# JackWoo0831/Yolov7-tracker

Measured on AMD Instinct MI355X. Metric: end-to-end fps (detect+track) YOLOv7-w6@1280 ByteTrack, higher is better.
Workload: dtype f16

## Files before the change

yolov7-tracker_amd/csrc/y7t_conv_p8.hip:

```cpp
#include "y7t_common.h"
#include "y7t_conv_common.h"
#include <stdlib.h>

namespace {

#if defined(Y7T_CONVSIM)
#define P8_VMCNT(n) cs_vmcnt(n)
#define P8_WAVE_SYNC() cs_wave_barrier(threadIdx.x >> 6)
#define P8_KEEP(a, b) ((void)0)
#else
#define P8_VMCNT(n) asm volatile("s_waitcnt vmcnt(" #n ")" ::: "memory")
#define P8_WAVE_SYNC() ((void)0)
#define P8_KEEP(a, b) asm volatile("" :: "v"(a), "v"(b))
#endif

struct P8 {
    static constexpr int BM = 256, BN = 256, BK = 64, NT = 512;
    static constexpr int ROWB = 128;
    static constexpr int HALF = 128 * ROWB;
    static constexpr int BUF = 4 * HALF;
    static constexpr int RING = 2 * BUF;
    static constexpr int BIAS = RING;
    static constexpr int LDS = RING + BN * 4;
    static constexpr unsigned OOB = 0xFF000000u;
};

template <int ACT, bool DUAL, int ABL = 0>
__global__ void __launch_bounds__(512, 2) k_conv1x1_p8(const Y7TConvArgs p) {
#if defined(__HIP_DEVICE_COMPILE__)
    using C = P8;
    extern __shared__ __attribute__((aligned(16))) char smem[];
    const int tid = threadIdx.x, lane = tid & 63, wave = tid >> 6;
    const int grp = wave >> 2, wq = wave & 3, l31 = lane & 31, hi32 = lane >> 5;

    int bid = blockIdx.x;
    if (p.xcd_swizzle) {
        const int nwg = gridDim.x, q = nwg >> 3, r = nwg & 7, xcd = bid & 7, idx = bid >> 3;
        bid = (xcd < r ? xcd * (q + 1) : r * (q + 1) + (xcd - r) * q) + idx;
    }
    const int n_tiles_n = p.Cout_pad / C::BN;
    const int tile_n = bid % n_tiles_n, tile_m = bid / n_tiles_n;
    const int m0 = tile_m * C::BM, n0 = tile_n * C::BN;
    const int nk = p.Cin / C::BK;

    const __amdgpu_buffer_rsrc_t xr = __builtin_amdgcn_make_buffer_rsrc((void*)p.in, 0, p.in_bytes, 0x00020000);
    const __amdgpu_buffer_rsrc_t wr = __builtin_amdgcn_make_buffer_rsrc((void*)p.w, 0, p.w_bytes, 0x00020000);
    const __amdgpu_buffer_rsrc_t br = __builtin_amdgcn_make_buffer_rsrc((void*)p.bias, 0, (unsigned)p.Cout_pad * 4u, 0x00020000);
    const __amdgpu_buffer_rsrc_t xr2 = __builtin_amdgcn_make_buffer_rsrc((void*)(DUAL ? p.in2 : p.in), 0, DUAL ? p.in2_bytes : p.in_bytes, 0x00020000);

    const int srow = wave * 8 + (lane >> 3);
    const int gch = (lane & 7) ^ ((srow >> 1) & 7);
    int xoff[2][2], xoff2[DUAL ? 2 : 1][2];
#pragma unroll
    for (int h = 0; h < 2; ++h)
#pragma unroll
        for (int rd = 0; rd < 2; ++rd) {
            const int m = m0 + rd * 128 + h * 64 + srow;
            xoff[h][rd] = (int)C::OOB;
            if (DUAL) xoff2[h][rd] = (int)C::OOB;
            if (m < p.M) {
                xoff[h][rd] = (m * p.ldin + p.cin_off + gch * 8) * 2;
                if (DUAL) {
                    const int HW = p.H * p.W, b = m / HW, rem = m - b * HW, y = rem / p.W, x = rem - y * p.W;
                    xoff2[h][rd] = (((b * (p.H >> 1) + (y >> 1)) * (p.W >> 1) + (x >> 1)) * p.ldin2 + p.cin2_off + gch * 8) * 2;
                }
            }
        }
    const int wvo = tile_n * nk * (2 * C::HALF) + wave * 1024 + lane * 16;

    bool in_loop = false;
    auto stage_p1 = [&](int h, int b, int T, int rd) __attribute__((always_inline)) {
        if ((ABL & 1) && in_loop) return;
        char* dst = smem + b * C::BUF + h * C::HALF + wave * 1024 + rd * 8192;
        const bool live = T < nk;
        const int ci = T * C::BK;
        const bool up = DUAL && live && ci >= p.up_c0 && ci < p.up_c0 + p.up_C;
        if (up) __builtin_amdgcn_raw_ptr_buffer_load_lds(xr2, (LDS_AS void*)dst, 16, xoff2[DUAL ? h : 0][rd], (ci - p.up_c0) * 2, 0, 0);
        else __builtin_amdgcn_raw_ptr_buffer_load_lds(xr, (LDS_AS void*)dst, 16, live ? xoff[h][rd] : (int)C::OOB, live ? ci * 2 : 0, 0, 0);
    };
    auto stage_c1 = [&](int h, int b, int T, int rd) __attribute__((always_inline)) {
        if ((ABL & 1) && in_loop) return;
        char* dst = smem + b * C::BUF + (2 + h) * C::HALF + wave * 1024 + rd * 8192;
        const bool live = T < nk;
        __builtin_amdgcn_raw_ptr_buffer_load_lds(wr, (LDS_AS void*)dst, 16, live ? wvo + h * C::HALF + rd * 8192 : (int)C::OOB, live ? T * (2 * C::HALF) : 0, 0, 0);
    };
    auto stage_p = [&](int h, int b, int T) __attribute__((always_inline)) { stage_p1(h, b, T, 0); stage_p1(h, b, T, 1); };
    auto stage_c = [&](int h, int b, int T) __attribute__((always_inline)) { stage_c1(h, b, T, 0); stage_c1(h, b, T, 1); };

    const int swl = (l31 >> 1) & 7;
    const int prow = (grp * 64 + l31) * C::ROWB, crow = (wq * 32 + l31) * C::ROWB;
    half8 pf[2][4], c0[4], c1[4];
    auto read_p = [&](int hP, int b) __attribute__((always_inline)) {
        if (ABL & 4) return;
#pragma unroll
        for (int j = 0; j < 2; ++j)
#pragma unroll
            for (int ks = 0; ks < 4; ++ks) pf[j][ks] = *(const half8*)(smem + b * C::BUF + hP * C::HALF + prow + j * 32 * C::ROWB + (((ks * 2 + hi32) ^ swl) << 4));
    };
    auto read_c = [&](half8 (&cf)[4], int hC, int b) __attribute__((always_inline)) {
        if (ABL & 4) return;
#pragma unroll
        for (int ks = 0; ks < 4; ++ks) cf[ks] = *(const half8*)(smem + b * C::BUF + (2 + hC) * C::HALF + crow + (((ks * 2 + hi32) ^ swl) << 4));
    };
    floatx16 acc[2][2][2];
    auto mma = [&](int hP, const half8 (&cf)[4], int hC) __attribute__((always_inline)) {
        if (!(ABL & 8)) __builtin_amdgcn_s_setprio(1);
#pragma unroll
        for (int ks = 0; ks < 4; ++ks)
#pragma unroll
            for (int j = 0; j < 2; ++j) {
                if (ABL & 2) P8_KEEP(cf[ks], pf[j][ks]);
                else acc[hP][j][hC] = __builtin_amdgcn_mfma_f32_32x32x16_f16(cf[ks], pf[j][ks], acc[hP][j][hC], 0, 0, 0);
            }
        if (!(ABL & 8)) __builtin_amdgcn_s_setprio(0);
    };

    __builtin_amdgcn_raw_ptr_buffer_load_lds(br, (LDS_AS void*)(smem + C::BIAS + wq * 256), 4, (n0 + wq * 64 + lane) * 4, 0, 0, 0);
    stage_p(0, 0, 0); stage_c(0, 0, 0); stage_c(1, 0, 0); stage_p(1, 0, 0); stage_p(0, 1, 1); stage_c(0, 1, 1);
    P8_VMCNT(8);
    __builtin_amdgcn_s_barrier();
#pragma unroll
    for (int hC = 0; hC < 2; ++hC)
#pragma unroll
        for (int g = 0; g < 4; ++g) {
            typedef __attribute__((ext_vector_type(4))) float float4v;
            const float4v bv = *(const float4v*)(smem + C::BIAS + (wq * 64 + hC * 32 + 8 * g + 4 * hi32) * 4);
#pragma unroll
            for (int hP = 0; hP < 2; ++hP)
#pragma unroll
                for (int j = 0; j < 2; ++j)
#pragma unroll
                    for (int e = 0; e < 4; ++e) acc[hP][j][hC][g * 4 + e] = bv[e];
        }
    if (grp == 1) __builtin_amdgcn_s_barrier();
    in_loop = true;
    if (ABL & 4) {
#pragma unroll
        for (int ks = 0; ks < 4; ++ks) { c0[ks] = c1[ks] = pf[0][ks] = pf[1][ks] = half8{1, 1, 1, 1, 1, 1, 1, 1}; }
    }

    auto ktile = [&](int T, auto bc) __attribute__((always_inline)) {
        constexpr int b = decltype(bc)::value;
        read_p(0, b); read_c(c0, 0, b);
        stage_c(1, b ^ 1, T + 1);
        P8_VMCNT(8);
        __builtin_amdgcn_s_barrier();
        mma(0, c0, 0);
        __builtin_amdgcn_s_barrier();
        read_c(c1, 1, b);
        stage_p(1, b ^ 1, T + 1);
        P8_VMCNT(8);
        __builtin_amdgcn_s_barrier();
        mma(0, c1, 1);
        __builtin_amdgcn_s_barrier();
        read_p(1, b);
        stage_p(0, b, T + 2);
        P8_VMCNT(8);
        __builtin_amdgcn_s_barrier();
        mma(1, c1, 1);
        __builtin_amdgcn_s_barrier();
        stage_c(0, b, T + 2);
        P8_VMCNT(8);
        __builtin_amdgcn_s_barrier();
        mma(1, c0, 0);
        __builtin_amdgcn_s_barrier();
    };
    for (int T = 0; T < nk; T += 2) {
        ktile(T, std::integral_constant<int, 0>{});
        if (T + 1 < nk) ktile(T + 1, std::integral_constant<int, 1>{});
    }
    if (grp == 0) __builtin_amdgcn_s_barrier();
    P8_VMCNT(0);
    __builtin_amdgcn_s_barrier();

    char* scr = smem + wave * 16384;
    typedef __attribute__((ext_vector_type(4))) unsigned uint4v;
#pragma unroll
    for (int hP = 0; hP < 2; ++hP)
#pragma unroll
        for (int j = 0; j < 2; ++j) {
            const int pl = hP * 64 + j * 32 + l31;
#pragma unroll
            for (int hC = 0; hC < 2; ++hC)
#pragma unroll
                for (int gp = 0; gp < 2; ++gp) {
                    unsigned w[2][2];
#pragma unroll
                    for (int gg = 0; gg < 2; ++gg) {
                        const int g = gp * 2 + gg;
                        float v[4];
#pragma unroll
                        for (int e = 0; e < 4; ++e) v[e] = act_t<ACT>(acc[hP][j][hC][g * 4 + e]);
                        typedef __attribute__((ext_vector_type(2))) _Float16 half2v;
                        half2v h0 = {(half_t)v[0], (half_t)v[1]}, h1 = {(half_t)v[2], (half_t)v[3]};
                        w[gg][0] = __builtin_bit_cast(unsigned, h0);
                        w[gg][1] = __builtin_bit_cast(unsigned, h1);
                    }
                    auto r0 = __builtin_amdgcn_permlane32_swap(w[0][0], w[1][0], false, false);
                    auto r1 = __builtin_amdgcn_permlane32_swap(w[0][1], w[1][1], false, false);
                    uint4v pk = {r0[0], r1[0], r0[1], r1[1]};
                    const int ch = hC * 4 + gp * 2 + hi32;
                    *(uint4v*)(scr + pl * 128 + ((ch ^ (pl & 7)) << 4)) = pk;
                }
        }
    P8_WAVE_SYNC();
    half_t* outp = (half_t*)p.out;
#pragma unroll 1
    for (int k0 = 0; k0 < 16; k0 += 8) {
        uint4v v[8];
#pragma unroll
        for (int k = 0; k < 8; ++k) {
            const int px = (k0 + k) * 8 + (lane >> 3), ch = lane & 7;
            v[k] = *(const uint4v*)(scr + px * 128 + ((ch ^ (px & 7)) << 4));
        }
        __builtin_amdgcn_sched_barrier(0);
#pragma unroll
        for (int k = 0; k < 8; ++k) {
            const int px = (k0 + k) * 8 + (lane >> 3), ch = lane & 7;
            const int m = m0 + grp * 128 + px, n = n0 + wq * 64 + ch * 8;
            if (m < p.M && n < p.Cout && !(ABL & 16)) *(uint4v*)(outp + (size_t)m * p.ldout + p.cout_off + n) = v[k];
        }
    }
#endif
}


template <int ACT, bool DUAL, bool DYN>
__global__ void __launch_bounds__(512, 2) k_conv1x1_p8p(const Y7TConvArgs p) {
#if defined(__HIP_DEVICE_COMPILE__)
    using C = P8;
    extern __shared__ __attribute__((aligned(16))) char smem[];
    const int tid = threadIdx.x, lane = tid & 63, wave = tid >> 6;
    const int grp = wave >> 2, wq = wave & 3, l31 = lane & 31, hi32 = lane >> 5;
    int bid = blockIdx.x;
    if (p.xcd_swizzle) {
        const int nwg = gridDim.x, q = nwg >> 3, r = nwg & 7, xcd = bid & 7, idx = bid >> 3;
        bid = (xcd < r ? xcd * (q + 1) : r * (q + 1) + (xcd - r) * q) + idx;
    }
    const int n_tiles_n = p.Cout_pad / C::BN, Gn = (int)gridDim.x / n_tiles_n;
    const int tile_n = bid % n_tiles_n, m_tiles = (p.M + C::BM - 1) / C::BM;
    int tile_m = bid / n_tiles_n;
    if (tile_m >= m_tiles) return;
    const int n0 = tile_n * C::BN, nk = p.Cin / C::BK;

    const __amdgpu_buffer_rsrc_t xr = __builtin_amdgcn_make_buffer_rsrc((void*)p.in, 0, p.in_bytes, 0x00020000);
    const __amdgpu_buffer_rsrc_t wr = __builtin_amdgcn_make_buffer_rsrc((void*)p.w, 0, p.w_bytes, 0x00020000);
    const __amdgpu_buffer_rsrc_t br = __builtin_amdgcn_make_buffer_rsrc((void*)p.bias, 0, (unsigned)p.Cout_pad * 4u, 0x00020000);
    const __amdgpu_buffer_rsrc_t xr2 = __builtin_amdgcn_make_buffer_rsrc((void*)(DUAL ? p.in2 : p.in), 0, DUAL ? p.in2_bytes : p.in_bytes, 0x00020000);

    const int srow = wave * 8 + (lane >> 3);
    const int gch = (lane & 7) ^ ((srow >> 1) & 7);
    struct Off { int x[2][2]; int x2[DUAL ? 2 : 1][2]; };
    auto offsets = [&](int m0, Off& o) __attribute__((always_inline)) {
#pragma unroll
        for (int h = 0; h < 2; ++h)
#pragma unroll
            for (int rd = 0; rd < 2; ++rd) {
                const int m = m0 + rd * 128 + h * 64 + srow;
                o.x[h][rd] = (int)C::OOB;
                if (DUAL) o.x2[h][rd] = (int)C::OOB;
                if (m < p.M) {
                    o.x[h][rd] = (m * p.ldin + p.cin_off + gch * 8) * 2;
                    if (DUAL) {
                        const int HW = p.H * p.W, b = m / HW, rem = m - b * HW, y = rem / p.W, x = rem - y * p.W;
                        o.x2[h][rd] = (((b * (p.H >> 1) + (y >> 1)) * (p.W >> 1) + (x >> 1)) * p.ldin2 + p.cin2_off + gch * 8) * 2;
                    }
                }
            }
    };
    Off cur, nxt;
    bool has_next = false;
    volatile int* const tkt = (volatile int*)(smem + C::LDS);
    int* const ctr = DYN ? p.tile_ctr + tile_n : nullptr;
    if (DYN && tid == 0) tkt[0] = atomicAdd(ctr, 1);
    const int wvo = tile_n * nk * (2 * C::HALF) + wave * 1024 + lane * 16;

    auto stage_p1 = [&](int h, int b, int T, int rd) __attribute__((always_inline)) {
        char* dst = smem + b * C::BUF + h * C::HALF + wave * 1024 + rd * 8192;
        const bool own = T < nk, live = own || has_next;
        const int ci = (own ? T : T - nk) * C::BK;
        const bool up = DUAL && live && ci >= p.up_c0 && ci < p.up_c0 + p.up_C;
        const int xo = own ? cur.x[h][rd] : nxt.x[h][rd];
        if (up) __builtin_amdgcn_raw_ptr_buffer_load_lds(xr2, (LDS_AS void*)dst, 16, own ? cur.x2[DUAL ? h : 0][rd] : nxt.x2[DUAL ? h : 0][rd], (ci - p.up_c0) * 2, 0, 0);
        else __builtin_amdgcn_raw_ptr_buffer_load_lds(xr, (LDS_AS void*)dst, 16, live ? xo : (int)C::OOB, live ? ci * 2 : 0, 0, 0);
    };
    auto stage_c1 = [&](int h, int b, int T, int rd) __attribute__((always_inline)) {
        char* dst = smem + b * C::BUF + (2 + h) * C::HALF + wave * 1024 + rd * 8192;
        const bool own = T < nk, live = own || has_next;
        const int Tw = own ? T : T - nk;
        __builtin_amdgcn_raw_ptr_buffer_load_lds(wr, (LDS_AS void*)dst, 16, live ? wvo + h * C::HALF + rd * 8192 : (int)C::OOB, live ? Tw * (2 * C::HALF) : 0, 0, 0);
    };
    auto stage_p = [&](int h, int b, int T) __attribute__((always_inline)) { stage_p1(h, b, T, 0); stage_p1(h, b, T, 1); };
    auto stage_c = [&](int h, int b, int T) __attribute__((always_inline)) { stage_c1(h, b, T, 0); stage_c1(h, b, T, 1); };

    const int swl = (l31 >> 1) & 7;
    const int prow = (grp * 64 + l31) * C::ROWB, crow = (wq * 32 + l31) * C::ROWB;
    half8 pf[2][4], c0[4], c1[4];
    auto read_p = [&](int hP, int b) __attribute__((always_inline)) {
#pragma unroll
        for (int j = 0; j < 2; ++j)
#pragma unroll
            for (int ks = 0; ks < 4; ++ks) pf[j][ks] = *(const half8*)(smem + b * C::BUF + hP * C::HALF + prow + j * 32 * C::ROWB + (((ks * 2 + hi32) ^ swl) << 4));
    };
    auto read_c = [&](half8 (&cf)[4], int hC, int b) __attribute__((always_inline)) {
#pragma unroll
        for (int ks = 0; ks < 4; ++ks) cf[ks] = *(const half8*)(smem + b * C::BUF + (2 + hC) * C::HALF + crow + (((ks * 2 + hi32) ^ swl) << 4));
    };
    floatx16 acc[2][2][2];
    auto mma = [&](int hP, const half8 (&cf)[4], int hC) __attribute__((always_inline)) {
        __builtin_amdgcn_s_setprio(1);
#pragma unroll
        for (int ks = 0; ks < 4; ++ks)
#pragma unroll
            for (int j = 0; j < 2; ++j) acc[hP][j][hC] = __builtin_amdgcn_mfma_f32_32x32x16_f16(cf[ks], pf[j][ks], acc[hP][j][hC], 0, 0, 0);
        __builtin_amdgcn_s_setprio(0);
    };
    auto ktile = [&](int T, auto bc) __attribute__((always_inline)) {
        constexpr int b = decltype(bc)::value;
        read_p(0, b); read_c(c0, 0, b);
        stage_c(1, b ^ 1, T + 1);
        P8_VMCNT(8);
        __builtin_amdgcn_s_barrier();
        mma(0, c0, 0);
        __builtin_amdgcn_s_barrier();
        read_c(c1, 1, b);
        stage_p(1, b ^ 1, T + 1);
        P8_VMCNT(8);
        __builtin_amdgcn_s_barrier();
        mma(0, c1, 1);
        __builtin_amdgcn_s_barrier();
        read_p(1, b);
        stage_p(0, b, T + 2);
        P8_VMCNT(8);
        __builtin_amdgcn_s_barrier();
        mma(1, c1, 1);
        __builtin_amdgcn_s_barrier();
        stage_c(0, b, T + 2);
        P8_VMCNT(8);
        __builtin_amdgcn_s_barrier();
        mma(1, c0, 0);
        __builtin_amdgcn_s_barrier();
    };

    offsets(tile_m * C::BM, cur);
    __builtin_amdgcn_raw_ptr_buffer_load_lds(br, (LDS_AS void*)(smem + C::BIAS + wq * 256), 4, (n0 + wq * 64 + lane) * 4, 0, 0, 0);
    stage_p(0, 0, 0); stage_c(0, 0, 0); stage_c(1, 0, 0); stage_p(1, 0, 0); stage_p(0, 1, 1); stage_c(0, 1, 1);
    P8_VMCNT(8);
    __builtin_amdgcn_s_barrier();
    typedef __attribute__((ext_vector_type(4))) unsigned uint4v;
    half_t* outp = (half_t*)p.out;
    char* const scr = smem + C::BUF + (wave < 4 ? 1 : 3) * C::HALF + (wave & 3) * 4096;
    for (int it = 0;; ++it) {
        const int m0 = tile_m * C::BM, tile_next = DYN ? Gn + __builtin_amdgcn_readfirstlane(tkt[it & 1]) : tile_m + Gn;
        has_next = tile_next < m_tiles;
        int fetched = 0;
        if (DYN && tid == 0 && has_next) {
#if defined(Y7T_CONVSIM)
            fetched = atomicAdd(ctr, 1);
#else
            asm volatile("global_atomic_add %0, %1, %2, off sc0" : "=v"(fetched) : "v"(ctr), "v"(1) : "memory");
#endif
        }
        if (has_next) offsets(tile_next * C::BM, nxt);
#pragma unroll
        for (int hC = 0; hC < 2; ++hC)
#pragma unroll
            for (int g = 0; g < 4; ++g) {
                typedef __attribute__((ext_vector_type(4))) float float4v;
                const float4v bv = *(const float4v*)(smem + C::BIAS + (wq * 64 + hC * 32 + 8 * g + 4 * hi32) * 4);
#pragma unroll
                for (int hP = 0; hP < 2; ++hP)
#pragma unroll
                    for (int j = 0; j < 2; ++j)
#pragma unroll
                        for (int e = 0; e < 4; ++e) acc[hP][j][hC][g * 4 + e] = bv[e];
            }
        if (grp == 1) __builtin_amdgcn_s_barrier();
        for (int T = 0; T < nk; T += 2) {
            ktile(T, std::integral_constant<int, 0>{});
            ktile(T + 1, std::integral_constant<int, 1>{});
        }
        if (grp == 0) __builtin_amdgcn_s_barrier();
        if (DYN && tid == 0 && has_next) tkt[(it + 1) & 1] = fetched;
#pragma unroll
        for (int hP = 0; hP < 2; ++hP)
#pragma unroll
            for (int j = 0; j < 2; ++j) {
#pragma unroll
                for (int hC = 0; hC < 2; ++hC)
#pragma unroll
                    for (int gp = 0; gp < 2; ++gp) {
                        unsigned w[2][2];
#pragma unroll
                        for (int gg = 0; gg < 2; ++gg) {
                            const int g = gp * 2 + gg;
                            float v[4];
#pragma unroll
                            for (int e = 0; e < 4; ++e) v[e] = act_t<ACT>(acc[hP][j][hC][g * 4 + e]);
                            typedef __attribute__((ext_vector_type(2))) _Float16 half2v;
                            half2v h0 = {(half_t)v[0], (half_t)v[1]}, h1 = {(half_t)v[2], (half_t)v[3]};
                            w[gg][0] = __builtin_bit_cast(unsigned, h0);
                            w[gg][1] = __builtin_bit_cast(unsigned, h1);
                        }
                        auto r0 = __builtin_amdgcn_permlane32_swap(w[0][0], w[1][0], false, false);
                        auto r1 = __builtin_amdgcn_permlane32_swap(w[0][1], w[1][1], false, false);
                        uint4v pk = {r0[0], r1[0], r0[1], r1[1]};
                        const int ch = hC * 4 + gp * 2 + hi32;
                        *(uint4v*)(scr + l31 * 128 + ((ch ^ (l31 & 7)) << 4)) = pk;
                    }
                P8_WAVE_SYNC();
                uint4v v4[4];
#pragma unroll
                for (int k = 0; k < 4; ++k) {
                    const int px = k * 8 + (lane >> 3), ch = lane & 7;
                    v4[k] = *(const uint4v*)(scr + px * 128 + ((ch ^ (px & 7)) << 4));
                }
                __builtin_amdgcn_sched_barrier(0);
#pragma unroll
                for (int k = 0; k < 4; ++k) {
                    const int px = k * 8 + (lane >> 3), ch = lane & 7;
                    const int m = m0 + grp * 128 + hP * 64 + j * 32 + px, n = n0 + wq * 64 + ch * 8;
                    if (m < p.M && n < p.Cout) *(uint4v*)(outp + (size_t)m * p.ldout + p.cout_off + n) = v4[k];
                }
                P8_WAVE_SYNC();
            }
        if (!has_next) break;
        __builtin_amdgcn_s_barrier();
        cur = nxt;
        tile_m = tile_next;
    }
    P8_VMCNT(0);
    if (DYN && tid == 0) {
        if (atomicAdd(p.tile_ctr + Y7T_TILE_CTR_DONE, 1) == (int)gridDim.x - 1) {
            for (int i = 0; i <= Y7T_TILE_CTR_DONE; ++i) p.tile_ctr[i] = 0;
        }
    }
#endif
}

}

int y7t_conv_p8_launch(const Y7TConvArgs& a, hipStream_t s) {
    using C = P8;
    bool ok = a.KH == 1 && a.KW == 1 && a.stride == 1 && a.pad == 0 && a.Cin % C::BK == 0 && a.K_pad == a.Cin && a.Cout_pad % C::BN == 0 && !a.out_f32 && !a.epi &&
              !(a.Cout & 7) && !(a.ldout & 7) && !(a.cout_off & 7) && !(a.ldin & 7) && !(a.cin_off & 7) && a.in_bytes <= C::OOB - (1u << 24) && a.Ho == a.H && a.Wo == a.W;
    if (a.up_C > 0) ok = ok && a.up_c0 % C::BK == 0 && a.up_C % C::BK == 0 && a.up_c0 + a.up_C <= a.Cin && !(a.H & 1) && !(a.W & 1) && !(a.ldin2 & 7) && !(a.cin2_off & 7) &&
                         a.in2_bytes <= C::OOB - (1u << 24);
    if (!ok) {
        y7t_set_error("conv: weights are in the 256 x 64 panel order (korder 7) but the layer is not a 1x1 / stride 1 convolution with Cin %% 64 == 0, Cout_pad %% 256 == 0 "
                      "and an aligned fp16 output (Cin=%d Cout=%d Cout_pad=%d ldout=%d cout_off=%d up=[%d,%d))", a.Cin, a.Cout, a.Cout_pad, a.ldout, a.cout_off, a.up_c0,
                      a.up_c0 + a.up_C);
        return Y7T_E_ARG;
    }
    static Y7TOncePerDevice attr;
    if (int e_ = y7t_once_per_device(attr, [&]() -> int {
#define P8_ATTR(ACT, DUAL) Y7T_HIP_CHECK(hipFuncSetAttribute((const void*)k_conv1x1_p8<ACT, DUAL>, hipFuncAttributeMaxDynamicSharedMemorySize, C::LDS));
        P8_ATTR(Y7T_ACT_NONE, false) P8_ATTR(Y7T_ACT_SILU, false) P8_ATTR(Y7T_ACT_LEAKY, false) P8_ATTR(Y7T_ACT_NONE, true) P8_ATTR(Y7T_ACT_SILU, true) P8_ATTR(Y7T_ACT_LEAKY, true)
#undef P8_ATTR
        return 0;
    })) return e_;
    const int grid = ((a.M + C::BM - 1) / C::BM) * (a.Cout_pad / C::BN);
    const bool dual = a.up_C > 0;
    static const int persist = y7t_exp_switch("Y7T_CONV_P8_PERSIST", 1);
    const int n_tiles_n = a.Cout_pad / C::BN, ncu = y7t_num_cus(), gp_ = (ncu / n_tiles_n) * n_tiles_n;
    if (persist && !a.ablate && ((a.Cin / C::BK) & 1) == 0 && gp_ > 0 && grid >= 2 * gp_) {
        static Y7TOncePerDevice attrp;
        if (int e_ = y7t_once_per_device(attrp, [&]() -> int {
#define P8P_ATTR(ACT, DUAL) Y7T_HIP_CHECK(hipFuncSetAttribute((const void*)k_conv1x1_p8p<ACT, DUAL, false>, hipFuncAttributeMaxDynamicSharedMemorySize, C::LDS + 16)); \
                            Y7T_HIP_CHECK(hipFuncSetAttribute((const void*)k_conv1x1_p8p<ACT, DUAL, true>, hipFuncAttributeMaxDynamicSharedMemorySize, C::LDS + 16));
            P8P_ATTR(Y7T_ACT_NONE, false) P8P_ATTR(Y7T_ACT_SILU, false) P8P_ATTR(Y7T_ACT_LEAKY, false) P8P_ATTR(Y7T_ACT_NONE, true) P8P_ATTR(Y7T_ACT_SILU, true) P8P_ATTR(Y7T_ACT_LEAKY, true)
#undef P8P_ATTR
            return 0;
        })) return e_;
        static const int dyn_env = y7t_switch("Y7T_CONV_WS_DYN", 1);
        const bool dyn = a.tile_ctr && dyn_env && n_tiles_n <= Y7T_TILE_CTR_DONE;
#define P8P_GO(ACT) \
        do { if (dual && dyn) hipLaunchKernelGGL((k_conv1x1_p8p<ACT, true, true>), dim3(gp_), dim3(C::NT), C::LDS + 16, s, a); \
             else if (dual) hipLaunchKernelGGL((k_conv1x1_p8p<ACT, true, false>), dim3(gp_), dim3(C::NT), C::LDS + 16, s, a); \
             else if (dyn) hipLaunchKernelGGL((k_conv1x1_p8p<ACT, false, true>), dim3(gp_), dim3(C::NT), C::LDS + 16, s, a); \
             else hipLaunchKernelGGL((k_conv1x1_p8p<ACT, false, false>), dim3(gp_), dim3(C::NT), C::LDS + 16, s, a); } while (0)
        if (a.act == Y7T_ACT_SILU) P8P_GO(Y7T_ACT_SILU);
        else if (a.act == Y7T_ACT_LEAKY) P8P_GO(Y7T_ACT_LEAKY);
        else P8P_GO(Y7T_ACT_NONE);
#undef P8P_GO
        Y7T_LAUNCH_CHECK();
        y7t_note_kernel("p8<256,256,64> 1x1%s", dual ? " upsample-on-read" : "");
        return 0;
    }
#if Y7T_ABLATE
    if (a.ablate && a.act == Y7T_ACT_SILU && !dual) {
#define P8_ABL(N) case N: Y7T_HIP_CHECK(hipFuncSetAttribute((const void*)k_conv1x1_p8<Y7T_ACT_SILU, false, N>, hipFuncAttributeMaxDynamicSharedMemorySize, C::LDS)); \
                          hipLaunchKernelGGL((k_conv1x1_p8<Y7T_ACT_SILU, false, N>), dim3(grid), dim3(C::NT), C::LDS, s, a); break;
        switch (a.ablate) { P8_ABL(1) P8_ABL(2) P8_ABL(4) P8_ABL(8) P8_ABL(16) P8_ABL(6) P8_ABL(7) default: y7t_set_error("conv: unknown p8 ablation %d", a.ablate); return Y7T_E_ARG; }
#undef P8_ABL
        Y7T_LAUNCH_CHECK();
        y7t_note_kernel("p8<256,256,64> 1x1 ablated");
        return 0;
    }
#endif
#define P8_GO(ACT) \
    do { if (dual) hipLaunchKernelGGL((k_conv1x1_p8<ACT, true>), dim3(grid), dim3(C::NT), C::LDS, s, a); \
         else hipLaunchKernelGGL((k_conv1x1_p8<ACT, false>), dim3(grid), dim3(C::NT), C::LDS, s, a); } while (0)
    if (a.act == Y7T_ACT_SILU) P8_GO(Y7T_ACT_SILU);
    else if (a.act == Y7T_ACT_LEAKY) P8_GO(Y7T_ACT_LEAKY);
    else P8_GO(Y7T_ACT_NONE);
#undef P8_GO
    Y7T_LAUNCH_CHECK();
    y7t_note_kernel("p8<256,256,64> 1x1%s", dual ? " upsample-on-read" : "");
    return 0;
}
```

Before: 2456.

## Interleave SiLU epilogue math into the last k-tile's MFMA gaps

For SiLU-activated 1x1 conv kernels, the last k-tile now applies the activation to already-final accumulator quadrants between MFMA issues. A compile-time micro-program table spreads the exp, rcp and multiply steps across the gaps of the 8 MFMAs per phase, and the epilogue skips those elements. This is meant to hide part of the epilogue's transcendental work behind matrix-core latency. The persistent kernel also moves bias re-initialization into the store loop and makes the wave index scalar via readfirstlane. The cost is added code complexity, scheduling barriers that constrain the compiler, and more register pressure from temporaries.

```diff
diff --git a/yolov7-tracker_amd/csrc/y7t_conv_p8.hip b/yolov7-tracker_amd/csrc/y7t_conv_p8.hip
--- a/yolov7-tracker_amd/csrc/y7t_conv_p8.hip
+++ b/yolov7-tracker_amd/csrc/y7t_conv_p8.hip
@@ -8,10 +8,12 @@
 #define P8_VMCNT(n) cs_vmcnt(n)
 #define P8_WAVE_SYNC() cs_wave_barrier(threadIdx.x >> 6)
 #define P8_KEEP(a, b) ((void)0)
+#define P8_PIN(x) ((void)0)
 #else
 #define P8_VMCNT(n) asm volatile("s_waitcnt vmcnt(" #n ")" ::: "memory")
 #define P8_WAVE_SYNC() ((void)0)
 #define P8_KEEP(a, b) asm volatile("" :: "v"(a), "v"(b))
+#define P8_PIN(x) asm volatile("" : "+v"(x))
 #endif
 
 struct P8 {
@@ -25,12 +27,68 @@
     static constexpr unsigned OOB = 0xFF000000u;
 };
 
+struct P8EA {
+    static constexpr int L = 4, G = 6;
+    static constexpr int PER_PHASE = L + G, N = 3 * PER_PHASE;
+    static_assert(L >= 0 && G >= 0 && PER_PHASE <= 32, "a phase may only touch quadrants that are final");
+    enum { EX, M1, RC, AD, M2 };
+    static constexpr int NOPS = 5 * (G + 3);
+    struct Tbl { signed char gap[NOPS], val[NOPS]; int last; };
+    static constexpr Tbl make() {
+        Tbl t{};
+        constexpr int dv[5] = {0, 1, -1, 0, -2}, cost[5] = {8, 4, 8, 4, 4};
+        int gap = 0, used = 0;
+        for (int o = 0; o < NOPS; ++o) {
+            const int k = o % 5, v = o / 5 - 1 + dv[k];
+            t.val[o] = (signed char)v;
+            t.gap[o] = -1;
+            if (v < 0 || v >= G) continue;
+            if (used + cost[k] > 24) { ++gap; used = 0; }
+            used += cost[k];
+            t.gap[o] = (signed char)gap;
+        }
+        t.last = gap;
+        return t;
+    }
+    static constexpr int index(int hP, int j, int hC, int e) { return ((hP == 0 ? hC : 3 - hC) * 2 + j) * 16 + e; }
+};
+static_assert(P8EA::make().last <= 7, "the micro-program of a phase fits the gaps of its 8 MFMAs");
+typedef floatx16 P8Acc[2][2][2];
+__device__ __forceinline__ float p8_ea_get(const P8Acc& acc, int n) { const int q = n >> 5; return acc[q >> 1][(n >> 4) & 1][q == 1 || q == 2][n & 15]; }
+__device__ __forceinline__ void p8_ea_set(P8Acc& acc, int n, float y) { const int q = n >> 5; acc[q >> 1][(n >> 4) & 1][q == 1 || q == 2][n & 15] = y; }
+__device__ __forceinline__ void p8_ea_load(P8Acc& acc, int ph) {
+#pragma unroll
+    for (int i = 0; i < P8EA::L; ++i) {
+        const int n = (ph - 1) * P8EA::PER_PHASE + i;
+        float y = act_t<Y7T_ACT_SILU>(p8_ea_get(acc, n));
+        P8_PIN(y);
+        p8_ea_set(acc, n, y);
+    }
+}
+__device__ __forceinline__ void p8_ea_gap(P8Acc& acc, float (&t)[P8EA::G > 0 ? P8EA::G : 1], int ph, int g) {
+    constexpr P8EA::Tbl tbl = P8EA::make();
+#pragma unroll
+    for (int o = 0; o < P8EA::NOPS; ++o) {
+        if (tbl.gap[o] != g) continue;
+        const int v = tbl.val[o], n = (ph - 1) * P8EA::PER_PHASE + P8EA::L + v;
+        switch (o % 5) {
+            case P8EA::M1: t[v] = -1.44269504088896f * p8_ea_get(acc, n); break;
+            case P8EA::EX: t[v] = __builtin_amdgcn_exp2f(t[v]); break;
+            case P8EA::AD: t[v] = 1.0f + t[v]; break;
+            case P8EA::RC: t[v] = __builtin_amdgcn_rcpf(t[v]); break;
+            default: t[v] = p8_ea_get(acc, n) * t[v]; break;
+        }
+        P8_PIN(t[v]);
+        if (o % 5 == P8EA::M2) p8_ea_set(acc, n, t[v]);
+    }
+}
+
 template <int ACT, bool DUAL, int ABL = 0>
 __global__ void __launch_bounds__(512, 2) k_conv1x1_p8(const Y7TConvArgs p) {
 #if defined(__HIP_DEVICE_COMPILE__)
     using C = P8;
     extern __shared__ __attribute__((aligned(16))) char smem[];
-    const int tid = threadIdx.x, lane = tid & 63, wave = tid >> 6;
+    const int tid = threadIdx.x, lane = tid & 63, wave = __builtin_amdgcn_readfirstlane(tid >> 6);
     const int grp = wave >> 2, wq = wave & 3, l31 = lane & 31, hi32 = lane >> 5;
 
     int bid = blockIdx.x;
@@ -102,7 +160,7 @@
 #pragma unroll
         for (int ks = 0; ks < 4; ++ks) cf[ks] = *(const half8*)(smem + b * C::BUF + (2 + hC) * C::HALF + crow + (((ks * 2 + hi32) ^ swl) << 4));
     };
-    floatx16 acc[2][2][2];
+    P8Acc acc;
     auto mma = [&](int hP, const half8 (&cf)[4], int hC) __attribute__((always_inline)) {
         if (!(ABL & 8)) __builtin_amdgcn_s_setprio(1);
 #pragma unroll
@@ -114,6 +172,25 @@
             }
         if (!(ABL & 8)) __builtin_amdgcn_s_setprio(0);
     };
+    constexpr bool EA = ACT == Y7T_ACT_SILU && ABL == 0 && P8EA::N > 0;
+    float eat[P8EA::G > 0 ? P8EA::G : 1];
+    auto mma_ea = [&](int hP, const half8 (&cf)[4], int hC, int ph) __attribute__((always_inline)) {
+        __builtin_amdgcn_s_setprio(1);
+#pragma unroll
+        for (int ks = 0; ks < 4; ++ks)
+#pragma unroll
+            for (int j = 0; j < 2; ++j) {
+                acc[hP][j][hC] = __builtin_amdgcn_mfma_f32_32x32x16_f16(cf[ks], pf[j][ks], acc[hP][j][hC], 0, 0, 0);
+                p8_ea_gap(acc, eat, ph, ks * 2 + j);
+                __builtin_amdgcn_sched_barrier(0);
+            }
+        __builtin_amdgcn_s_setprio(0);
+    };
+    auto ea_load = [&](int ph) __attribute__((always_inline)) {
+        __builtin_amdgcn_sched_barrier(0);
+        p8_ea_load(acc, ph);
+        __builtin_amdgcn_sched_barrier(0);
+    };
 
     __builtin_amdgcn_raw_ptr_buffer_load_lds(br, (LDS_AS void*)(smem + C::BIAS + wq * 256), 4, (n0 + wq * 64 + lane) * 4, 0, 0, 0);
     stage_p(0, 0, 0); stage_c(0, 0, 0); stage_c(1, 0, 0); stage_p(1, 0, 0); stage_p(0, 1, 1); stage_c(0, 1, 1);
@@ -139,8 +216,9 @@
         for (int ks = 0; ks < 4; ++ks) { c0[ks] = c1[ks] = pf[0][ks] = pf[1][ks] = half8{1, 1, 1, 1, 1, 1, 1, 1}; }
     }
 
-    auto ktile = [&](int T, auto bc) __attribute__((always_inline)) {
-        constexpr int b = decltype(bc)::value;
+    auto ktile = [&](int T, auto bc, auto lc) __attribute__((always_inline)) {
+        const int b = bc;
+        constexpr bool LAST = EA && decltype(lc)::value;
         read_p(0, b); read_c(c0, 0, b);
         stage_c(1, b ^ 1, T + 1);
         P8_VMCNT(8);
@@ -149,25 +227,32 @@
         __builtin_amdgcn_s_barrier();
         read_c(c1, 1, b);
         stage_p(1, b ^ 1, T + 1);
-        P8_VMCNT(8);
-        __builtin_amdgcn_s_barrier();
-        mma(0, c1, 1);
+        if (LAST) ea_load(1);
+        P8_VMCNT(8);
+        __builtin_amdgcn_s_barrier();
+        if (LAST) mma_ea(0, c1, 1, 1); else mma(0, c1, 1);
         __builtin_amdgcn_s_barrier();
         read_p(1, b);
         stage_p(0, b, T + 2);
-        P8_VMCNT(8);
-        __builtin_amdgcn_s_barrier();
-        mma(1, c1, 1);
+        if (LAST) ea_load(2);
+        P8_VMCNT(8);
+        __builtin_amdgcn_s_barrier();
+        if (LAST) mma_ea(1, c1, 1, 2); else mma(1, c1, 1);
         __builtin_amdgcn_s_barrier();
         stage_c(0, b, T + 2);
-        P8_VMCNT(8);
-        __builtin_amdgcn_s_barrier();
-        mma(1, c0, 0);
-        __builtin_amdgcn_s_barrier();
-    };
-    for (int T = 0; T < nk; T += 2) {
-        ktile(T, std::integral_constant<int, 0>{});
-        if (T + 1 < nk) ktile(T + 1, std::integral_constant<int, 1>{});
+        if (LAST) ea_load(3);
+        P8_VMCNT(8);
+        __builtin_amdgcn_s_barrier();
+        if (LAST) mma_ea(1, c0, 0, 3); else mma(1, c0, 0);
+        __builtin_amdgcn_s_barrier();
+    };
+    {
+        constexpr std::integral_constant<int, 0> B0{};
+        constexpr std::integral_constant<int, 1> B1{};
+        int T = 0;
+        for (; T + 2 < nk; T += 2) { ktile(T, B0, std::false_type{}); ktile(T + 1, B1, std::false_type{}); }
+        if (T + 1 < nk) { ktile(T, B0, std::false_type{}); ++T; }
+        ktile(T, T & 1, std::true_type{});
     }
     if (grp == 0) __builtin_amdgcn_s_barrier();
     P8_VMCNT(0);
@@ -190,7 +275,7 @@
                         const int g = gp * 2 + gg;
                         float v[4];
 #pragma unroll
-                        for (int e = 0; e < 4; ++e) v[e] = act_t<ACT>(acc[hP][j][hC][g * 4 + e]);
+                        for (int e = 0; e < 4; ++e) v[e] = EA && P8EA::index(hP, j, hC, g * 4 + e) < P8EA::N ? acc[hP][j][hC][g * 4 + e] : act_t<ACT>(acc[hP][j][hC][g * 4 + e]);
                         typedef __attribute__((ext_vector_type(2))) _Float16 half2v;
                         half2v h0 = {(half_t)v[0], (half_t)v[1]}, h1 = {(half_t)v[2], (half_t)v[3]};
                         w[gg][0] = __builtin_bit_cast(unsigned, h0);
@@ -230,7 +315,7 @@
 #if defined(__HIP_DEVICE_COMPILE__)
     using C = P8;
     extern __shared__ __attribute__((aligned(16))) char smem[];
-    const int tid = threadIdx.x, lane = tid & 63, wave = tid >> 6;
+    const int tid = threadIdx.x, lane = tid & 63, wave = __builtin_amdgcn_readfirstlane(tid >> 6);
     const int grp = wave >> 2, wq = wave & 3, l31 = lane & 31, hi32 = lane >> 5;
     int bid = blockIdx.x;
     if (p.xcd_swizzle) {
@@ -306,7 +391,7 @@
 #pragma unroll
         for (int ks = 0; ks < 4; ++ks) cf[ks] = *(const half8*)(smem + b * C::BUF + (2 + hC) * C::HALF + crow + (((ks * 2 + hi32) ^ swl) << 4));
     };
-    floatx16 acc[2][2][2];
+    P8Acc acc;
     auto mma = [&](int hP, const half8 (&cf)[4], int hC) __attribute__((always_inline)) {
         __builtin_amdgcn_s_setprio(1);
 #pragma unroll
@@ -315,8 +400,28 @@
             for (int j = 0; j < 2; ++j) acc[hP][j][hC] = __builtin_amdgcn_mfma_f32_32x32x16_f16(cf[ks], pf[j][ks], acc[hP][j][hC], 0, 0, 0);
         __builtin_amdgcn_s_setprio(0);
     };
-    auto ktile = [&](int T, auto bc) __attribute__((always_inline)) {
+    constexpr bool EA = ACT == Y7T_ACT_SILU && P8EA::N > 0;
+    float eat[P8EA::G > 0 ? P8EA::G : 1];
+    auto mma_ea = [&](int hP, const half8 (&cf)[4], int hC, int ph) __attribute__((always_inline)) {
+        __builtin_amdgcn_s_setprio(1);
+#pragma unroll
+        for (int ks = 0; ks < 4; ++ks)
+#pragma unroll
+            for (int j = 0; j < 2; ++j) {
+                acc[hP][j][hC] = __builtin_amdgcn_mfma_f32_32x32x16_f16(cf[ks], pf[j][ks], acc[hP][j][hC], 0, 0, 0);
+                p8_ea_gap(acc, eat, ph, ks * 2 + j);
+                __builtin_amdgcn_sched_barrier(0);
+            }
+        __builtin_amdgcn_s_setprio(0);
+    };
+    auto ea_load = [&](int ph) __attribute__((always_inline)) {
+        __builtin_amdgcn_sched_barrier(0);
+        p8_ea_load(acc, ph);
+        __builtin_amdgcn_sched_barrier(0);
+    };
+    auto ktile = [&](int T, auto bc, auto lc) __attribute__((always_inline)) {
         constexpr int b = decltype(bc)::value;
+        constexpr bool LAST = EA && decltype(lc)::value;
         read_p(0, b); read_c(c0, 0, b);
         stage_c(1, b ^ 1, T + 1);
         P8_VMCNT(8);
@@ -325,20 +430,23 @@
         __builtin_amdgcn_s_barrier();
         read_c(c1, 1, b);
         stage_p(1, b ^ 1, T + 1);
-        P8_VMCNT(8);
-        __builtin_amdgcn_s_barrier();
-        mma(0, c1, 1);
+        if (LAST) ea_load(1);
+        P8_VMCNT(8);
+        __builtin_amdgcn_s_barrier();
+        if (LAST) mma_ea(0, c1, 1, 1); else mma(0, c1, 1);
         __builtin_amdgcn_s_barrier();
         read_p(1, b);
         stage_p(0, b, T + 2);
-        P8_VMCNT(8);
-        __builtin_amdgcn_s_barrier();
-        mma(1, c1, 1);
+        if (LAST) ea_load(2);
+        P8_VMCNT(8);
+        __builtin_amdgcn_s_barrier();
+        if (LAST) mma_ea(1, c1, 1, 2); else mma(1, c1, 1);
         __builtin_amdgcn_s_barrier();
         stage_c(0, b, T + 2);
-        P8_VMCNT(8);
-        __builtin_amdgcn_s_barrier();
-        mma(1, c0, 0);
+        if (LAST) ea_load(3);
+        P8_VMCNT(8);
+        __builtin_amdgcn_s_barrier();
+        if (LAST) mma_ea(1, c0, 0, 3); else mma(1, c0, 0);
         __builtin_amdgcn_s_barrier();
     };
 
@@ -350,6 +458,17 @@
     typedef __attribute__((ext_vector_type(4))) unsigned uint4v;
     half_t* outp = (half_t*)p.out;
     char* const scr = smem + C::BUF + (wave < 4 ? 1 : 3) * C::HALF + (wave & 3) * 4096;
+    auto bias_init = [&](int hP, int j) __attribute__((always_inline)) {
+#pragma unroll
+        for (int hC = 0; hC < 2; ++hC)
+#pragma unroll
+            for (int g = 0; g < 4; ++g) {
+                typedef __attribute__((ext_vector_type(4))) float float4v;
+                const float4v bv = *(const float4v*)(smem + C::BIAS + (wq * 64 + hC * 32 + 8 * g + 4 * hi32) * 4);
+#pragma unroll
+                for (int e = 0; e < 4; ++e) acc[hP][j][hC][g * 4 + e] = bv[e];
+            }
+    };
     for (int it = 0;; ++it) {
         const int m0 = tile_m * C::BM, tile_next = DYN ? Gn + __builtin_amdgcn_readfirstlane(tkt[it & 1]) : tile_m + Gn;
         has_next = tile_next < m_tiles;
@@ -362,23 +481,20 @@
 #endif
         }
         if (has_next) offsets(tile_next * C::BM, nxt);
-#pragma unroll
-        for (int hC = 0; hC < 2; ++hC)
-#pragma unroll
-            for (int g = 0; g < 4; ++g) {
-                typedef __attribute__((ext_vector_type(4))) float float4v;
-                const float4v bv = *(const float4v*)(smem + C::BIAS + (wq * 64 + hC * 32 + 8 * g + 4 * hi32) * 4);
-#pragma unroll
-                for (int hP = 0; hP < 2; ++hP)
-#pragma unroll
-                    for (int j = 0; j < 2; ++j)
-#pragma unroll
-                        for (int e = 0; e < 4; ++e) acc[hP][j][hC][g * 4 + e] = bv[e];
-            }
+        if (it == 0) {
+#pragma unroll
+            for (int hP = 0; hP < 2; ++hP)
+#pragma unroll
+                for (int j = 0; j < 2; ++j) bias_init(hP, j);
+        }
         if (grp == 1) __builtin_amdgcn_s_barrier();
-        for (int T = 0; T < nk; T += 2) {
-            ktile(T, std::integral_constant<int, 0>{});
-            ktile(T + 1, std::integral_constant<int, 1>{});
+        {
+            constexpr std::integral_constant<int, 0> B0{};
+            constexpr std::integral_constant<int, 1> B1{};
+            int T = 0;
+            for (; T + 2 < nk; T += 2) { ktile(T, B0, std::false_type{}); ktile(T + 1, B1, std::false_type{}); }
+            ktile(T, B0, std::false_type{});
+            ktile(T + 1, B1, std::true_type{});
         }
         if (grp == 0) __builtin_amdgcn_s_barrier();
         if (DYN && tid == 0 && has_next) tkt[(it + 1) & 1] = fetched;
@@ -396,7 +512,7 @@
                             const int g = gp * 2 + gg;
                             float v[4];
 #pragma unroll
-                            for (int e = 0; e < 4; ++e) v[e] = act_t<ACT>(acc[hP][j][hC][g * 4 + e]);
+                            for (int e = 0; e < 4; ++e) v[e] = EA && P8EA::index(hP, j, hC, g * 4 + e) < P8EA::N ? acc[hP][j][hC][g * 4 + e] : act_t<ACT>(acc[hP][j][hC][g * 4 + e]);
                             typedef __attribute__((ext_vector_type(2))) _Float16 half2v;
                             half2v h0 = {(half_t)v[0], (half_t)v[1]}, h1 = {(half_t)v[2], (half_t)v[3]};
                             w[gg][0] = __builtin_bit_cast(unsigned, h0);
@@ -408,6 +524,7 @@
                         const int ch = hC * 4 + gp * 2 + hi32;
                         *(uint4v*)(scr + l31 * 128 + ((ch ^ (l31 & 7)) << 4)) = pk;
                     }
+                bias_init(hP, j);
                 P8_WAVE_SYNC();
                 uint4v v4[4];
 #pragma unroll
```

New measurement: 2469, median of 6. About the same (+0.6%).
